# wkvong/multimodal-baby

Measured on AMD Instinct MI355X. Metric: image-text pairs/sec, CVCL ResNeXt+embed 224², bs256, 1/2/4/8 MI355X, higher is better.
Workload: dtype bf16; 1 GPU; C2 = BASELINE configs[1]: CVCL saycam_contrastive, frozen random-init ResNeXt-50 32x4d (BN train mode) + embedding mean-pool text encoder, E=512, L2-normalised, fixed tau 0.07, 224x224 frames + 3-word utterances; full step = fwd + InfoNCE + bwd(fc, embedding) + AdamW; per_gpu_batch=256, global_batch=256, negatives=local (single GPU), parallelism=dp1, trunk_streams=2

## Files before the change

multimodal-baby_amd/csrc/cvcl_common.h:

```cpp
#pragma once
#include <hip/hip_runtime.h>
#include <stdint.h>

#include "../../include/cvcl_hip.h"

typedef __bf16 bf16_t;
typedef __bf16 bf16x4 __attribute__((ext_vector_type(4)));
typedef __bf16 bf16x8 __attribute__((ext_vector_type(8)));
typedef float f32x4 __attribute__((ext_vector_type(4)));
typedef float f32x16 __attribute__((ext_vector_type(16)));
typedef unsigned int u32x4 __attribute__((ext_vector_type(4)));
typedef unsigned int u32x2 __attribute__((ext_vector_type(2)));

#define CVCL_WAVE 64

void cvcl_set_error(const char* fmt, ...);

int cvcl_gemm_cu_share();
bool cvcl_env_on(const char* name);

bool cvcl_prof_on();
void* cvcl_prof_begin(void* stream, int cls);
void cvcl_prof_end(void* handle, void* stream);
struct CvclProfScope {
    void* h; void* s;
    CvclProfScope(void* stream, int cls) : h(cvcl_prof_begin(stream, cls)), s(stream) {}
    ~CvclProfScope() { cvcl_prof_end(h, s); }
};

#ifdef __cplusplus
#include <atomic>
struct CvclLdsAttr {
    std::atomic<unsigned long long> devs{0};
    static int dev() { int d = 0; (void)hipGetDevice(&d); return d & 63; }
    bool ready() const { return (devs.load(std::memory_order_acquire) >> dev()) & 1ull; }
    void mark() { if (!ready()) devs.fetch_or(1ull << dev(), std::memory_order_release); }
};
static inline int cvcl_raise_lds_limit(CvclLdsAttr& attr, const void* kernel, int bytes, const char* entry) {
    if (attr.ready()) return CVCL_OK;
    if (hipFuncSetAttribute(kernel, hipFuncAttributeMaxDynamicSharedMemorySize, bytes) != hipSuccess) {
        cvcl_set_error("%s: cannot raise the dynamic LDS limit (%d bytes)", entry, bytes);
        return CVCL_ELAUNCH;
    }
    return CVCL_OK;
}
#endif

#define CVCL_CHECK_ARG(cond, ...)                \
    do {                                         \
        if (!(cond)) {                           \
            cvcl_set_error(__VA_ARGS__);         \
            return CVCL_EINVAL;                  \
        }                                        \
    } while (0)

#define CVCL_LAUNCH_CHECK()                                                    \
    do {                                                                       \
        hipError_t e_ = hipGetLastError();                                     \
        if (e_ != hipSuccess) {                                                \
            cvcl_set_error("%s:%d launch failed: %s", __FILE__, __LINE__,      \
                           hipGetErrorString(e_));                             \
            return CVCL_ELAUNCH;                                               \
        }                                                                      \
    } while (0)

__host__ __device__ static inline int cvcl_div_up(long a, long b) { return (int)((a + b - 1) / b); }

static inline int cvcl_grid(long items, int per_block, int cap) {
    const long g = (items + per_block - 1) / per_block;
    return (int)(g < 1 ? 1 : (g > cap ? cap : g));
}
static inline bool cvcl_aligned16(const void* p) { return ((uintptr_t)p & 15) == 0; }

static inline bool cvcl_dtype_plain(int d) { return d == CVCL_F32 || d == CVCL_BF16; }
static inline bool cvcl_dtype_trunk(int d) { return cvcl_dtype_plain(d) || d == CVCL_F32X3; }
static inline int cvcl_storage_dtype(int d) { return d == CVCL_F32X3 ? CVCL_F32 : d; }
#define CVCL_CHECK_DTYPE(d, fn) CVCL_CHECK_ARG(cvcl_dtype_plain(d), "%s: dtype %d is not accepted here (CVCL_F32 / CVCL_BF16)", fn, (int)(d))
#define CVCL_CHECK_DTYPE_TRUNK(d, fn) CVCL_CHECK_ARG(cvcl_dtype_trunk(d), "%s: unknown dtype %d", fn, (int)(d))

static inline bool cvcl_stats_rows_fit(const cvcl_gemm_args* a, int rows) {
    return !a->stats || a->stats_rows == CVCL_STATS_ACCUMULATE || a->stats_rows >= rows;
}
const char* cvcl_gemm8w_refusal(int epi, const cvcl_gemm_args* a, bool direct);
bool cvcl_gemm_pro_takes(const cvcl_gemm_args* a, bool stats);

constexpr int kSplitTerms = 6;
constexpr int kSplitParts = kSplitTerms == 3 ? 2 : 3;
int cvcl_gemm_split(const cvcl_gemm_args* a, void* stream);
int cvcl_gemm_split_stats_rows(int M, int N);
size_t cvcl_split_dense_bytes(long elems);
int cvcl_pack_split_dense(const float* w, void* out, long elems, void* stream);
size_t cvcl_split_conv_bytes(int stem, int cout);
int cvcl_pack_split_conv(int stem, const float* w, void* out, int cout, int cg, void* stream);
int cvcl_stem_split_stats_rows(int B, int H, int W);
int cvcl_gconv_split_stats_rows(int B, int H, int W, int C, int stride);
int cvcl_stem_split(const float* x, const void* w, float* y, float* stats, int stats_rows, const float* centre, int B, int H, int W,
                    void* stream);
int cvcl_gconv_split(const float* x, const float* a_scale, const float* a_shift, float act_floor, const void* w, float* y, float* stats,
                     int stats_rows, const float* centre, int B, int H, int W, int C, int cg, int stride, void* stream);

#ifdef __HIPCC__
template <typename T> struct ElemTraits;
template <> struct ElemTraits<float> {
    static constexpr int kPerChunk = 4;
    __device__ static inline float to_f(float v) { return v; }
    __device__ static inline float from_f(float v) { return v; }
};
template <> struct ElemTraits<bf16_t> {
    static constexpr int kPerChunk = 8;
    __device__ static inline float to_f(bf16_t v) { return (float)v; }
    __device__ static inline bf16_t from_f(float v) { return (bf16_t)v; }
};

template <typename T> struct Chunk;
template <> struct Chunk<float> {
    f32x4 v;
    __device__ inline void load(const float* p) { v = *reinterpret_cast<const f32x4*>(p); }
    __device__ inline void store(float* p) const { *reinterpret_cast<f32x4*>(p) = v; }
    __device__ inline void zero() { v = f32x4{0.f, 0.f, 0.f, 0.f}; }
    __device__ inline float get(int i) const { return v[i]; }
    __device__ inline void set(int i, float f) { v[i] = f; }
};
template <> struct Chunk<bf16_t> {
    bf16x8 v;
    __device__ inline void load(const bf16_t* p) { v = *reinterpret_cast<const bf16x8*>(p); }
    __device__ inline void store(bf16_t* p) const { *reinterpret_cast<bf16x8*>(p) = v; }
    __device__ inline void zero() {
        u32x4 z = {0u, 0u, 0u, 0u};
        v = __builtin_bit_cast(bf16x8, z);
    }
    __device__ inline float get(int i) const { return (float)v[i]; }
    __device__ inline void set(int i, float f) { v[i] = (bf16_t)f; }
};

typedef float f32x2 __attribute__((ext_vector_type(2)));
typedef __bf16 bf16x2 __attribute__((ext_vector_type(2)));
typedef short s16x2 __attribute__((ext_vector_type(2)));
__device__ __forceinline__ f32x2 widen2(unsigned u) {
    return f32x2{__builtin_bit_cast(float, u << 16), __builtin_bit_cast(float, u & 0xffff0000u)};
}
__device__ __forceinline__ float dot2c_bf16(float acc, unsigned a, unsigned b) {
    asm("v_dot2c_f32_bf16 %0, %1, %2" : "+v"(acc) : "v"(a), "v"(b));
    return acc;
}
template <int CTRL> __device__ __forceinline__ float dpp_quad_f32(float v) {
    return __builtin_bit_cast(float, __builtin_amdgcn_update_dpp(0, __builtin_bit_cast(int, v), CTRL, 0xf, 0xf, true));
}
__device__ __forceinline__ unsigned round2(f32x2 v) { return __builtin_bit_cast(unsigned, __builtin_convertvector(v, bf16x2)); }
__device__ __forceinline__ unsigned relu2(unsigned pair) {
    return __builtin_bit_cast(unsigned, __builtin_elementwise_max(__builtin_bit_cast(s16x2, pair), s16x2{0, 0}));
}

template <typename V> __device__ __forceinline__ void stream_store(V v, V* dst) { __builtin_nontemporal_store(v, dst); }

__device__ inline float wave_sum(float v) {
#pragma unroll
    for (int o = 32; o > 0; o >>= 1) v += __shfl_xor(v, o, 64);
    return v;
}
__device__ inline double wave_sum(double v) {
#pragma unroll
    for (int o = 32; o > 0; o >>= 1) v += __shfl_xor(v, o, 64);
    return v;
}
__device__ inline float wave_max(float v) {
#pragma unroll
    for (int o = 32; o > 0; o >>= 1) v = fmaxf(v, __shfl_xor(v, o, 64));
    return v;
}
__device__ __forceinline__ bool cvcl_better(float s, int i, float t, int j) { return s > t || (s == t && i < j); }
__device__ inline float block_sum(float v, float* scratch) {
    v = wave_sum(v);
    const int lane = threadIdx.x & 63, w = threadIdx.x >> 6, nw = (blockDim.x + 63) >> 6;
    __syncthreads();
    if (lane == 0) scratch[w] = v;
    __syncthreads();
    float r = 0.f;
    for (int i = 0; i < nw; ++i) r += scratch[i];
    return r;
}
__device__ inline float block_max(float v, float* scratch) {
    v = wave_max(v);
    const int lane = threadIdx.x & 63, w = threadIdx.x >> 6, nw = (blockDim.x + 63) >> 6;
    __syncthreads();
    if (lane == 0) scratch[w] = v;
    __syncthreads();
    float r = -INFINITY;
    for (int i = 0; i < nw; ++i) r = fmaxf(r, scratch[i]);
    return r;
}

constexpr int kBnAccRows = 8;
constexpr double kBnAccScale = 16777216.0;
__device__ __forceinline__ int cvcl_xcc_id() { return __builtin_amdgcn_s_getreg((3 << 11) | 20) & 7; }
constexpr long long kBnAccPoison = 1LL << 62;
constexpr float kBnAccMaxPartial = 268435456.f;
__device__ __forceinline__ void cvcl_bn_acc_add(float* stats_as_acc, int N, int n, float s, float q) {
    long long* row = reinterpret_cast<long long*>(stats_as_acc) + (long)cvcl_xcc_id() * 2 * N;
    if (fabsf(s) < kBnAccMaxPartial && fabsf(q) < kBnAccMaxPartial) {
        __hip_atomic_fetch_add(row + n, __double2ll_rn((double)s * kBnAccScale), __ATOMIC_RELAXED, __HIP_MEMORY_SCOPE_AGENT);
        __hip_atomic_fetch_add(row + N + n, __double2ll_rn((double)q * kBnAccScale), __ATOMIC_RELAXED, __HIP_MEMORY_SCOPE_AGENT);
    } else {
        __hip_atomic_fetch_max(row + N + n, kBnAccPoison, __ATOMIC_RELAXED, __HIP_MEMORY_SCOPE_AGENT);
    }
}
__device__ __forceinline__ void cvcl_bn_stats_out(float* stats, int acc_mode, long row, int N, int n, float s, float q) {
    if (acc_mode) cvcl_bn_acc_add(stats, N, n, s, q);
    else {
        stats[(row * 2 + 0) * N + n] = s;
        stats[(row * 2 + 1) * N + n] = q;
    }
}

__device__ inline float bn_ema(float r, float x, float m) { return fmaf(m, x, (1.f - m) * r); }

struct BnSrc {
    const long long* acc;
    int C;
    double count;
    const float* gamma; const float* beta; const float* centre;
    float* running_mean; float* running_var; int64_t* nbt;
    float momentum, eps;
    float* moments; int moments_ld;
    float* scale_out; float* shift_out;
};

template <int NCH>
__device__ __forceinline__ void bn_slice_affine(const BnSrc& b, int c0, bool publish, float* sc_out, float* sh_out) {
    const int c = threadIdx.x;
    if (c < NCH) {
        const int ch = c0 + c;
        long long v[2 * kBnAccRows];
#pragma unroll
        for (int r = 0; r < kBnAccRows; ++r) {
            v[2 * r] = b.acc[((long)r * 2 + 0) * b.C + ch];
            v[2 * r + 1] = b.acc[((long)r * 2 + 1) * b.C + ch];
        }
        long long S = 0, Q = 0;
        bool poisoned = false;
#pragma unroll
        for (int r = 0; r < kBnAccRows; ++r) { S += v[2 * r]; Q += v[2 * r + 1]; poisoned |= v[2 * r + 1] >= kBnAccPoison || v[2 * r + 1] < 0; }
        const double s = (double)S * (1.0 / kBnAccScale), q = (double)Q * (1.0 / kBnAccScale);
        const double mean = s / b.count;
        double var = q / b.count - mean * mean;
        if (var < 0.0) var = 0.0;
        if (poisoned) var = __builtin_nan("");
        const float sc = b.gamma[ch] / sqrtf((float)var + b.eps);
        const float sh = b.beta[ch] - (float)mean * sc;
        sc_out[c] = sc;
        sh_out[c] = sh;
        if (publish) {
            if (b.scale_out) { b.scale_out[ch] = sc; b.shift_out[ch] = sh; }
            const double unbiased = b.count > 1.0 ? var * b.count / (b.count - 1.0) : var;
            const float true_mean = b.centre ? (float)(mean + (double)b.centre[ch]) : (float)mean;
            if (b.moments) {
                b.moments[ch] = true_mean;
                b.moments[b.moments_ld + ch] = (float)unbiased;
            } else if (b.running_mean) {
                b.running_mean[ch] = bn_ema(b.running_mean[ch], true_mean, b.momentum);
                b.running_var[ch] = bn_ema(b.running_var[ch], (float)unbiased, b.momentum);
            }
        }
    }
    if (publish && !b.moments && b.nbt && c0 == 0 && threadIdx.x == 0) *b.nbt += 1;
    __syncthreads();
}

int cvcl_conv1x1_gram_src(const void* A, int lda, long M, int K, const float* a_scale, const float* a_shift, const BnSrc* src, int a_relu,
                          void* workspace, size_t workspace_bytes, const double** gram_out, void* stream);

template <int UN, typename ACC, typename F>
__device__ inline ACC ordered_sum(int n, F load) {
    ACC acc = (ACC)0;
    for (int i0 = 0; i0 < n; i0 += UN) {
        ACC v[UN];
#pragma unroll
        for (int u = 0; u < UN; ++u) v[u] = (ACC)load(min(i0 + u, n - 1));
#pragma unroll
        for (int u = 0; u < UN; ++u)
            if (i0 + u < n) acc += v[u];
    }
    return acc;
}

__device__ inline float gelu_erf_fast(float v) {
    const float x = fabsf(v) * 0.70710678118654752440f;
    const float t = __builtin_amdgcn_rcpf(fmaf(0.3275911f, x, 1.f));
    float poly = fmaf(1.061405429f, t, -1.453152027f);
    poly = fmaf(poly, t, 1.421413741f);
    poly = fmaf(poly, t, -0.284496736f);
    poly = fmaf(poly, t, 0.254829592f);
    poly *= t;
    const float e = __builtin_amdgcn_exp2f(-x * x * 1.4426950408889634f);
    const float erf_abs = fmaf(-poly, e, 1.f);
    return 0.5f * v * (1.f + copysignf(erf_abs, v));
}
__device__ inline float gelu_bf16out(float v) {
    const float u = fminf(v * v, 36.f);
    float p = fmaf(u, -0.0007030378797f * -1.4426950408889634f, 0.07401131995f * -1.4426950408889634f);
    p = fmaf(p, u, 1.595015736f * -1.4426950408889634f);
    const float e = __builtin_amdgcn_exp2f(v * p);
    return v * __builtin_amdgcn_rcpf(1.f + e);
}
__device__ inline f32x2 gelu_bf16out2(f32x2 v) {
    f32x2 u = v * v;
    u = f32x2{fminf(u[0], 36.f), fminf(u[1], 36.f)};
// ... 63 lines not shown
```

multimodal-baby_amd/csrc/gemm8w_kernel.h:

```cpp
#pragma once
#include <type_traits>

#include "cvcl_common.h"

namespace g8w {

constexpr int BN = 256;
constexpr int BK = 32;
constexpr int NSTAGE = 4;
constexpr int A_BYTES = 16384;
constexpr int STAGE_BYTES = 2 * A_BYTES;
constexpr int STG_BYTES = 2048;
constexpr int ACC_OFF = NSTAGE * STAGE_BYTES + 8 * STG_BYTES;
constexpr int LDS_BYTES = 160 * 1024;
constexpr int MAX_BIAS_N = (LDS_BYTES - ACC_OFF) / 4;

struct Dev {
    const bf16_t* A; const bf16_t* W; bf16_t* C; const bf16_t* R;
    const float* bias; float* stats;
    int stats_acc;
    const float* ln_stats; const float* ln_colsum; float* row_part;
    const float* centre;
    int M, N, K, lda, ldw, ldc, ldr, act;
    int tiles_m, grid_m, ncol;
    int gs, g_hw, g_wo, g_hi, g_wi;
    int a_rows;
};

__device__ __forceinline__ void glds16(const bf16_t* src, char* lds_wave_base) {
    __builtin_amdgcn_global_load_lds((const void __attribute__((address_space(1)))*)src,
                                     (void __attribute__((address_space(3)))*)lds_wave_base, 16, 0, 0);
}

__device__ __forceinline__ int swz(int g) { return (0x78 >> (2 * g)) & 3; }

template <int N> __device__ __forceinline__ void wait_vm() {
    static_assert(N >= 0 && N <= 63, "vmcnt is a 6-bit field");
    asm volatile("s_waitcnt vmcnt(%0)" ::"n"(N) : "memory");
}

__device__ __forceinline__ void wait_vm_value(int n, u32x4& v) {
#define CVCL_W(N) case N: asm volatile("s_waitcnt vmcnt(" #N ")" : "+v"(v) : : "memory"); break;
    switch (n) {
        CVCL_W(0) CVCL_W(1) CVCL_W(2) CVCL_W(3) CVCL_W(4) CVCL_W(5) CVCL_W(6) CVCL_W(7) CVCL_W(8) CVCL_W(9) CVCL_W(10) CVCL_W(11)
        CVCL_W(12) CVCL_W(13) CVCL_W(14) CVCL_W(15) CVCL_W(16) CVCL_W(17) CVCL_W(18) CVCL_W(19) CVCL_W(20) CVCL_W(21) CVCL_W(22)
        CVCL_W(23) CVCL_W(24) CVCL_W(25) CVCL_W(26) CVCL_W(27) CVCL_W(28) CVCL_W(29) CVCL_W(30) CVCL_W(31) CVCL_W(32) CVCL_W(33)
        CVCL_W(34) CVCL_W(35) CVCL_W(36) CVCL_W(37) CVCL_W(38) CVCL_W(39) CVCL_W(40)
        default: asm volatile("s_waitcnt vmcnt(0)" : "+v"(v) : : "memory"); break;
    }
#undef CVCL_W
}

template <int MI, int EPI, bool LNF, int ACT = CVCL_ACT_NONE>
__global__ __launch_bounds__(512, 2) void gemm8w_kernel(Dev p) {
    constexpr int BM = MI * 32;
    static_assert(!LNF || EPI >= 1, "LNF goes with the linear epilogues");
    static_assert(ACT == CVCL_ACT_NONE || EPI == 1, "activations go with the bias epilogue");
    constexpr int ESTORES = MI * 2 + (LNF && EPI == 2 ? MI * 2 : 0);
    extern __shared__ __attribute__((aligned(16))) char smem[];
    const int tid = threadIdx.x, lane = tid & 63;
    const int wave = __builtin_amdgcn_readfirstlane(tid >> 6);
    const int wm = wave >> 2, wn = wave & 3;

    constexpr bool LIN = EPI >= 1, RES = EPI == 2;
    constexpr bool FLAT = LIN;
    const int b = blockIdx.x;
    const int G = gridDim.x;
    int ti, tj, nt;
    int L0 = 0;
    const int cpx = G >> 3;
    auto decode = [&](int L, int& i_out, int& j_out) __attribute__((always_inline)) {
        const int per = p.grid_m * p.ncol;
        const int sr = L / per, rem = L - sr * per;
        const int ah = min(p.grid_m, p.tiles_m - sr * p.grid_m);
        const int col = rem / ah;
        i_out = sr * p.grid_m + (rem - col * ah);
        j_out = (sr & 1) ? p.ncol - 1 - col : col;
    };
    if constexpr (FLAT) {
        const int xcd = b & 7;
        const int total = p.tiles_m * p.ncol;
        const int S0 = (int)(((long)xcd * total) >> 3), S1 = (int)(((long)(xcd + 1) * total) >> 3);
        L0 = S0 + (b >> 3);
        nt = L0 < S1 ? (S1 - L0 + cpx - 1) / cpx : 0;
        ti = 0; tj = 0;
        if (nt > 0) decode(L0, ti, tj);
    } else {
        const int xcd = b & 7, s = b >> 3;
        tj = s % p.ncol;
        ti = (s / p.ncol) * 8 + xcd;
        nt = ti < p.tiles_m ? (p.tiles_m - ti + p.grid_m - 1) / p.grid_m : 0;
    }
    const int KS = p.K / BK;
    const int S = nt * KS;
    if (S == 0) {
        if (EPI == 0 && p.stats && !p.stats_acc && ti < p.grid_m && tid < BN) {
            p.stats[((long)ti * 2 + 0) * p.N + tj * BN + tid] = 0.f;
            p.stats[((long)ti * 2 + 1) * p.N + tj * BN + tid] = 0.f;
        }
        return;
    }
    const int step_i = p.grid_m;

    const bf16_t* __restrict__ A = p.A;
    const bf16_t* __restrict__ W = p.W;

    const int srow = lane >> 2;
    const int slog = (lane & 3) ^ swz((lane >> 4) & 3);
    unsigned w_off[2], a_raw[2];
#pragma unroll
    for (int j = 0; j < 2; ++j) {
        w_off[j] = (unsigned)(tj * BN + (wave * 2 + j) * 16 + srow) * (unsigned)p.ldw + slog * 8;
        int r = (wave * 2 + j) * 16 + srow;
        if (r >= BM) r = BM - 1;
        a_raw[j] = (unsigned)(ti * BM + r) * (unsigned)p.lda + slog * 8;
    }
    auto gathered = [&](int i_tile, int j) __attribute__((always_inline)) -> unsigned {
        int r = (wave * 2 + j) * 16 + srow;
        if (r >= BM) r = BM - 1;
        const unsigned m = (unsigned)min(i_tile * BM + r, p.M - 1);
        const unsigned bi = m / (unsigned)p.g_hw, rem = m - bi * (unsigned)p.g_hw;
        const unsigned oy = rem / (unsigned)p.g_wo, ox = rem - oy * (unsigned)p.g_wo;
        return ((bi * p.g_hi + oy * p.gs) * p.g_wi + ox * p.gs) * (unsigned)p.lda + slog * 8;
    };
    if (p.gs > 1) { a_raw[0] = gathered(ti, 0); a_raw[1] = gathered(ti, 1); }
    const unsigned a_unit = (unsigned)BM * (unsigned)p.lda;
    const unsigned a_lim = (unsigned)(p.a_rows - 1) * (unsigned)p.lda + 24;
    int l_t = 0, l_ks = 0, l_j = tj, l_i = ti;
    auto issue = [&](int buf) __attribute__((always_inline)) {
        char* base = smem + buf * STAGE_BYTES + wave * 2048;
        const int k0 = l_ks * BK;
#pragma unroll
        for (int j = 0; j < 2; ++j) glds16(A + min(a_raw[j], a_lim) + k0, base + j * 1024);
#pragma unroll
        for (int j = 0; j < 2; ++j) glds16(W + w_off[j] + k0, base + A_BYTES + j * 1024);
    };
    auto advance = [&]() __attribute__((always_inline)) {
        if constexpr (LNF && EPI == 1) {
            if (l_ks == 0 && wave < 4) {
                char* dst = smem + ACC_OFF + (l_t & 1) * 4096 + wave * 1024;
                const float* src = wave == 0 ? p.bias + l_j * BN + lane * 4 : wave == 1 ? p.ln_colsum + l_j * BN + lane * 4
                                 : p.ln_stats + (long)min(l_i * BM + (wave - 2) * 128 + lane * 2, (p.M - 1) & ~1) * 2;
                __builtin_amdgcn_global_load_lds((const void __attribute__((address_space(1)))*)src,
                                                 (void __attribute__((address_space(3)))*)dst, 16, 0, 0);
            }
        }
        if (++l_ks == KS) {
            l_ks = 0;
            if (l_t + 1 < nt) {
                ++l_t;
                if constexpr (FLAT) {
                    decode(L0 + l_t * cpx, l_i, l_j);
#pragma unroll
                    for (int j = 0; j < 2; ++j) {
                        const int rw = (wave * 2 + j) * 16 + srow;
                        a_raw[j] = (unsigned)(l_i * BM + min(rw, BM - 1)) * (unsigned)p.lda + slog * 8;
                        w_off[j] = (unsigned)(l_j * BN + rw) * (unsigned)p.ldw + slog * 8;
                    }
                } else {
                    l_i += step_i;
#pragma unroll
                    for (int j = 0; j < 2; ++j) {
                        if (p.gs > 1) a_raw[j] = gathered(l_i, j);
                        else a_raw[j] += (unsigned)step_i * a_unit;
                    }
                }
            }
        }
    };

    const int f_off = (lane & 15) * 64 + (((lane >> 4) ^ swz((lane >> 2) & 3)) << 4);
    const int a_base = wm * (BM / 2) * 64 + f_off;
    const int w_base = A_BYTES + wn * 64 * 64 + f_off;

    bf16x8 fa[2][MI], fw[2][4];
    f32x4 acc[4][MI];
    auto read_frags = [&](int buf, auto P) __attribute__((always_inline)) {
        constexpr int q = decltype(P)::value;
        const char* sb = smem + buf * STAGE_BYTES;
#pragma unroll
        for (int ni = 0; ni < 4; ++ni) fw[q][ni] = *reinterpret_cast<const bf16x8*>(sb + w_base + ni * 1024);
#pragma unroll
        for (int mi = 0; mi < MI; ++mi) fa[q][mi] = *reinterpret_cast<const bf16x8*>(sb + a_base + mi * 1024);
    };
    auto mma_half = [&](auto P, auto HALF) __attribute__((always_inline)) {
        constexpr int q = decltype(P)::value, h = decltype(HALF)::value;
#pragma unroll
        for (int ni = 2 * h; ni < 2 * h + 2; ++ni)
#pragma unroll
            for (int mi = 0; mi < MI; ++mi)
                acc[ni][mi] = __builtin_amdgcn_mfma_f32_16x16x32_bf16(fw[q][ni], fa[q][mi], acc[ni][mi], 0, 0, 0);
    };
#pragma unroll
    for (int ni = 0; ni < 4; ++ni)
#pragma unroll
        for (int mi = 0; mi < MI; ++mi) acc[ni][mi] = f32x4{0.f, 0.f, 0.f, 0.f};

    float* lds_acc = reinterpret_cast<float*>(smem + ACC_OFF);
    if constexpr (LIN && LNF && EPI == 1) {
    } else if constexpr (LIN) {
        for (int i = tid; i < p.N; i += 512) lds_acc[i] = p.bias ? p.bias[i] : 0.f;
    } else {
        lds_acc[tid] = 0.f;
        lds_acc[tid + 512] = 0.f;
// ... 226 lines not shown
```

multimodal-baby_amd/csrc/gemm_pro.hip:

```cpp
#include <cstdlib>

#include "cvcl_common.h"

namespace {

constexpr int PM = 64;
constexpr int PN = 256;

struct ProDev {
    const bf16_t* A; const bf16_t* W; bf16_t* C; const bf16_t* R;
    const float* a_scale; const float* a_shift; const float* c_scale; const float* c_shift; const float* r_scale; const float* r_shift;
    float* stats;
    int stats_acc;
    const float* centre;
    int M, N, lda, ldw, ldc, ldr;
    int tiles;
    const bf16_t* A2; const bf16_t* W2; const float* centre2;
    int lda2, ldw2;
};

enum { PRO_STATS = 0, PRO_STORE = 1, PRO_TAIL = 2, PRO_TAIL_DS = 3 };
constexpr int K2 = 64, KT2 = 2;
constexpr int X2BUF = PM * K2 * 2;

template <int KT> constexpr int pro_lds_bytes() { return 2 * PM * KT * 64 + 8 * 4096 + 6 * PN * 4 + 2 * 256 * 4 + 2 * X2BUF; }

template <int KT, int MODE, int D>
__global__ __launch_bounds__(512, 2) void gemm_pro_kernel(ProDev p) {
    constexpr bool TAIL = MODE == PRO_TAIL || MODE == PRO_TAIL_DS, DS = MODE == PRO_TAIL_DS;
    constexpr int K = KT * 32;
    constexpr int PITCH = K * 2;
    constexpr int CPR = K / 8;
    constexpr int NCH = PM * CPR / 512;
    constexpr int RPP = 512 / CPR;
    constexpr int ABUF = PM * PITCH;
    extern __shared__ __attribute__((aligned(16))) char smem[];
    const int tid = threadIdx.x, lane = tid & 63;
    const int wave = __builtin_amdgcn_readfirstlane(tid >> 6);
    const int wm = wave >> 2, wn = wave & 3;
    const int n0 = blockIdx.y * PN;

    bf16x8 fw[4][KT];
#pragma unroll
    for (int ni = 0; ni < 4; ++ni)
#pragma unroll
        for (int ks = 0; ks < KT; ++ks)
            fw[ni][ks] = *reinterpret_cast<const bf16x8*>(p.W + (long)(n0 + wn * 64 + ni * 16 + (lane & 15)) * p.ldw + ks * 32 + (lane >> 4) * 8);

    const int s_c = tid % CPR, s_r = tid / CPR;
    constexpr bool AFF_LDS = KT == 8;
    float* in_aff = reinterpret_cast<float*>(smem + 2 * ABUF + 8 * 4096 + 6 * PN * 4);
    char* x2buf = smem + 2 * ABUF + 8 * 4096 + 6 * PN * 4 + 2 * 256 * 4;
    const bool plain = p.a_scale == nullptr;
    const short fl = plain ? (short)-32768 : (short)0;
    const s16x2 floor2 = s16x2{fl, fl};
    f32x2 sc[4], sh[4];
#pragma unroll
    for (int e = 0; e < 4; ++e) { sc[e] = f32x2{1.f, 1.f}; sh[e] = f32x2{0.f, 0.f}; }
    if constexpr (AFF_LDS) {
        if (tid < K) { in_aff[tid] = plain ? 1.f : p.a_scale[tid]; in_aff[K + tid] = plain ? 0.f : p.a_shift[tid]; }
        __syncthreads();
    } else if (!plain) {
#pragma unroll
        for (int e = 0; e < 4; ++e) {
            sc[e] = f32x2{p.a_scale[s_c * 8 + 2 * e], p.a_scale[s_c * 8 + 2 * e + 1]};
            sh[e] = f32x2{p.a_shift[s_c * 8 + 2 * e], p.a_shift[s_c * 8 + 2 * e + 1]};
        }
    }
    u32x4 araw[D][NCH];
    auto load_a = [&](int tile, int slot) __attribute__((always_inline)) {
#pragma unroll
        for (int i = 0; i < NCH; ++i) {
            int m = tile * PM + s_r + RPP * i;
            if (m >= p.M) m = p.M - 1;
            araw[slot][i] = *reinterpret_cast<const u32x4*>(p.A + (long)m * p.lda + s_c * 8);
        }
    };
    auto stage_a = [&](int buf, int slot) __attribute__((always_inline)) {
        char* dst = smem + buf * ABUF;
        if constexpr (AFF_LDS) {
#pragma unroll
            for (int e = 0; e < 4; ++e) {
                sc[e] = *reinterpret_cast<const f32x2*>(in_aff + s_c * 8 + 2 * e);
                sh[e] = *reinterpret_cast<const f32x2*>(in_aff + K + s_c * 8 + 2 * e);
            }
        }
#pragma unroll
        for (int i = 0; i < NCH; ++i) {
            const int r = s_r + RPP * i;
            u32x4 v;
#pragma unroll
            for (int e = 0; e < 4; ++e) {
                const unsigned y = round2(__builtin_elementwise_fma(widen2(araw[slot][i][e]), sc[e], sh[e]));
                v[e] = __builtin_bit_cast(unsigned, __builtin_elementwise_max(__builtin_bit_cast(s16x2, y), floor2));
            }
            *reinterpret_cast<u32x4*>(dst + r * PITCH + ((s_c ^ (r & 15)) << 4)) = v;
        }
    };
    const int f_row = lane & 15, f_kc = lane >> 4;

    const int r_chunk = lane & 7, r_row0 = lane >> 3;
    float* aff = reinterpret_cast<float*>(smem + 2 * ABUF + 8 * 4096);
    if (tid < PN) aff[4 * PN + tid] = p.centre ? -p.centre[n0 + tid] : 0.f;
    if constexpr (DS) { if (tid < PN) aff[5 * PN + tid] = p.centre2 ? -p.centre2[n0 + tid] : 0.f; }
    const float* cen = aff + 4 * PN + wn * 64 + (lane >> 4) * 4;
    bf16x8 fw2[DS ? 4 : 1][DS ? KT2 : 1];
    u32x4 x2raw[DS ? D : 1];
    const int x_r = tid >> 3, x_c = tid & 7;
    if constexpr (DS) {
#pragma unroll
        for (int ni = 0; ni < 4; ++ni)
#pragma unroll
            for (int ks = 0; ks < KT2; ++ks)
                fw2[ni][ks] = *reinterpret_cast<const bf16x8*>(p.W2 + (long)(n0 + wn * 64 + ni * 16 + (lane & 15)) * p.ldw2 + ks * 32 + (lane >> 4) * 8);
    }
    auto load_x2 = [&](int tile, int slot) __attribute__((always_inline)) {
        int m = tile * PM + x_r;
        if (m >= p.M) m = p.M - 1;
        x2raw[slot] = *reinterpret_cast<const u32x4*>(p.A2 + (long)m * p.lda2 + x_c * 8);
    };
    auto stage_x2 = [&](int buf, int slot) __attribute__((always_inline)) {
        *reinterpret_cast<u32x4*>(x2buf + buf * X2BUF + x_r * 128 + ((x_c ^ (x_r & 7)) << 4)) = x2raw[slot];
    };
    if constexpr (TAIL) {
        if (tid < PN) {
            aff[tid] = p.c_scale[n0 + tid];
            aff[PN + tid] = p.c_shift[n0 + tid];
            aff[2 * PN + tid] = p.r_scale ? p.r_scale[n0 + tid] : 1.f;
            aff[3 * PN + tid] = p.r_scale ? p.r_shift[n0 + tid] : 0.f;
        }
    }
    bf16x8 rres[4];
    auto load_r = [&](int tile) __attribute__((always_inline)) {
#pragma unroll
        for (int j = 0; j < 4; ++j) {
            int m = tile * PM + wm * 32 + j * 8 + r_row0;
            if (m >= p.M) m = p.M - 1;
            rres[j] = *reinterpret_cast<const bf16x8*>(p.R + (long)m * p.ldr + n0 + wn * 64 + r_chunk * 8);
        }
    };
    f32x2 st_sum[8], st_sq[8];
#pragma unroll
    for (int e = 0; e < 8; ++e) { st_sum[e] = f32x2{0.f, 0.f}; st_sq[e] = f32x2{0.f, 0.f}; }

    char* stg = smem + 2 * ABUF + wave * 4096;
    const int e_row = lane & 15, e_wchunk = lane >> 5, e_wsub = ((lane >> 4) & 1) * 8;

    const int first = blockIdx.x;
    const int G = gridDim.x;
#pragma unroll
    for (int d = 0; d < D; ++d)
        if (first + d * G < p.tiles) {
            load_a(first + d * G, d);
            if constexpr (DS) load_x2(first + d * G, d);
        }
    if constexpr (MODE == PRO_TAIL) {
        if (first < p.tiles) load_r(first);
    }
    f32x4 acc[4][2];
    auto tile_stats = [&](int m0) __attribute__((always_inline)) {
#pragma unroll
        for (int mi = 0; mi < 2; ++mi) {
            const unsigned keep = m0 + mi * 16 + e_row < p.M ? 0xffffffffu : 0u;
#pragma unroll
            for (int ni = 0; ni < 4; ++ni)
#pragma unroll
                for (int h = 0; h < 2; ++h) {
                    const f32x2 f = widen2(round2(f32x2{acc[ni][mi][2 * h], acc[ni][mi][2 * h + 1]}) & keep);
                    st_sum[ni * 2 + h] += f;
                    st_sq[ni * 2 + h] = __builtin_elementwise_fma(f, f, st_sq[ni * 2 + h]);
                }
        }
    };
    int buf = 0;
    for (int tile = first; tile < p.tiles;) {
#pragma unroll
      for (int slot = 0; slot < D; ++slot) {
        if (tile >= p.tiles) break;
        stage_a(buf, slot);
        if constexpr (DS) stage_x2(buf, slot);
        __syncthreads();
        const int next = tile + G;
        if (tile + D * G < p.tiles) {
            load_a(tile + D * G, slot);
            if constexpr (DS) load_x2(tile + D * G, slot);
        }
        unsigned r2[DS ? 4 : 1][2][2];
        if constexpr (DS) {
            f32x4 acc2[4][2];
            const float* cen2 = aff + 5 * PN + wn * 64 + (lane >> 4) * 4;
#pragma unroll
            for (int ni = 0; ni < 4; ++ni) {
                const f32x4 c4 = *reinterpret_cast<const f32x4*>(cen2 + ni * 16);
#pragma unroll
                for (int mi = 0; mi < 2; ++mi) acc2[ni][mi] = c4;
            }
            const char* xb = x2buf + buf * X2BUF + (wm * 32 + f_row) * 128;
#pragma unroll
            for (int ks = 0; ks < KT2; ++ks) {
                bf16x8 fx[2];
#pragma unroll
                for (int mi = 0; mi < 2; ++mi)
                    fx[mi] = *reinterpret_cast<const bf16x8*>(xb + mi * 16 * 128 + (((ks * 4 + f_kc) ^ (f_row & 7)) << 4));
#pragma unroll
                for (int ni = 0; ni < 4; ++ni)
#pragma unroll
                    for (int mi = 0; mi < 2; ++mi)
                        acc2[ni][mi] = __builtin_amdgcn_mfma_f32_16x16x32_bf16(fw2[ni][ks], fx[mi], acc2[ni][mi], 0, 0, 0);
            }
#pragma unroll
            for (int ni = 0; ni < 4; ++ni)
#pragma unroll
                for (int mi = 0; mi < 2; ++mi) {
                    r2[ni][mi][0] = round2(f32x2{acc2[ni][mi][0], acc2[ni][mi][1]});
                    r2[ni][mi][1] = round2(f32x2{acc2[ni][mi][2], acc2[ni][mi][3]});
                }
        }
#pragma unroll
        for (int ni = 0; ni < 4; ++ni) {
            const f32x4 c4 = *reinterpret_cast<const f32x4*>(cen + ni * 16);
#pragma unroll
            for (int mi = 0; mi < 2; ++mi) acc[ni][mi] = c4;
        }
        const char* ab = smem + buf * ABUF + (wm * 32 + f_row) * PITCH;
#pragma unroll
        for (int ks = 0; ks < KT; ++ks) {
            bf16x8 fa[2];
#pragma unroll
            for (int mi = 0; mi < 2; ++mi)
                fa[mi] = *reinterpret_cast<const bf16x8*>(ab + mi * 16 * PITCH + (((ks * 4 + f_kc) ^ f_row) << 4));
#pragma unroll
            for (int ni = 0; ni < 4; ++ni)
#pragma unroll
                for (int mi = 0; mi < 2; ++mi)
                    acc[ni][mi] = __builtin_amdgcn_mfma_f32_16x16x32_bf16(fw[ni][ks], fa[mi], acc[ni][mi], 0, 0, 0);
        }
        const int m0 = tile * PM + wm * 32;
        if constexpr (MODE == PRO_STATS) {
            tile_stats(m0);
        } else if constexpr (DS) {
#pragma unroll
            for (int ni = 0; ni < 4; ++ni) {
                const float* t = aff + wn * 64 + ni * 16 + (lane >> 4) * 4;
                const f32x4 cs = *reinterpret_cast<const f32x4*>(t), cb = *reinterpret_cast<const f32x4*>(t + PN);
                const f32x4 rs = *reinterpret_cast<const f32x4*>(t + 2 * PN), rb = *reinterpret_cast<const f32x4*>(t + 3 * PN);
#pragma unroll
                for (int mi = 0; mi < 2; ++mi) {
                    bf16x4 q;
#pragma unroll
                    for (int e = 0; e < 4; ++e) {
                        const float y = fmaf((float)(bf16_t)acc[ni][mi][e], cs[e], cb[e]);
                        const float idv = fmaf(widen2(r2[ni][mi][e >> 1])[e & 1], rs[e], rb[e]);
                        q[e] = (bf16_t)fmaxf(y + idv, 0.f);
                    }
                    const int row = mi * 16 + e_row, chunk = ni * 2 + e_wchunk;
                    *reinterpret_cast<bf16x4*>(stg + row * 128 + ((chunk ^ ((row >> 1) & 7)) << 4) + e_wsub) = q;
                }
            }
#pragma unroll
            for (int j = 0; j < 4; ++j) {
                const int row = j * 8 + r_row0;
                const bf16x8 v = *reinterpret_cast<const bf16x8*>(stg + row * 128 + ((r_chunk ^ ((row >> 1) & 7)) << 4));
                const int m = m0 + row, n = n0 + wn * 64 + r_chunk * 8;
                if (m < p.M) stream_store(v, reinterpret_cast<bf16x8*>(p.C + (long)m * p.ldc + n));
            }
        } else {
#pragma unroll
            for (int mi = 0; mi < 2; ++mi)
#pragma unroll
                for (int ni = 0; ni < 4; ++ni) {
                    const bf16x4 q = {(bf16_t)acc[ni][mi][0], (bf16_t)acc[ni][mi][1], (bf16_t)acc[ni][mi][2], (bf16_t)acc[ni][mi][3]};
                    const int row = mi * 16 + e_row, chunk = ni * 2 + e_wchunk;
                    *reinterpret_cast<bf16x4*>(stg + row * 128 + ((chunk ^ ((row >> 1) & 7)) << 4) + e_wsub) = q;
                }
            float cs[8], cb[8], rs[8], rb[8];
            if constexpr (MODE == PRO_TAIL) {
                const float* t = aff + wn * 64 + r_chunk * 8;
#pragma unroll
                for (int e = 0; e < 8; ++e) { cs[e] = t[e]; cb[e] = t[PN + e]; rs[e] = t[2 * PN + e]; rb[e] = t[3 * PN + e]; }
            }
#pragma unroll
            for (int j = 0; j < 4; ++j) {
                const int row = j * 8 + r_row0;
                bf16x8 v = *reinterpret_cast<const bf16x8*>(stg + row * 128 + ((r_chunk ^ ((row >> 1) & 7)) << 4));
                const int m = m0 + row, n = n0 + wn * 64 + r_chunk * 8;
                if (m < p.M) {
                    if constexpr (MODE == PRO_TAIL) {
                        const bf16x8 r = rres[j];
#pragma unroll
                        for (int e = 0; e < 8; ++e) {
                            const float y = fmaf((float)v[e], cs[e], cb[e]);
                            const float idv = fmaf((float)r[e], rs[e], rb[e]);
                            v[e] = (bf16_t)fmaxf(y + idv, 0.f);
                        }
                    } else {
                        const u32x4 u = __builtin_bit_cast(u32x4, v);
#pragma unroll
                        for (int e = 0; e < 4; ++e) {
                            const f32x2 f = widen2(u[e]);
                            st_sum[e] += f;
                            st_sq[e] = __builtin_elementwise_fma(f, f, st_sq[e]);
                        }
                    }
                    stream_store(v, reinterpret_cast<bf16x8*>(p.C + (long)m * p.ldc + n));
                }
            }
            if constexpr (MODE == PRO_TAIL) {
                if (next < p.tiles) load_r(next);
            }
        }
        buf ^= 1;
        tile += G;
      }
    }

    if (!TAIL && p.stats) {
        __syncthreads();
        float* red = (float*)smem;
        if constexpr (MODE == PRO_STATS) {
#pragma unroll
            for (int e = 0; e < 8; ++e)
#pragma unroll
                for (int h = 0; h < 2; ++h)
#pragma unroll
                    for (int o = 1; o < 16; o <<= 1) {
                        st_sum[e][h] += __shfl_xor(st_sum[e][h], o, 64);
                        st_sq[e][h] += __shfl_xor(st_sq[e][h], o, 64);
                    }
            if ((lane & 15) == 0) {
#pragma unroll
                for (int ni = 0; ni < 4; ++ni)
#pragma unroll
                    for (int e = 0; e < 4; ++e) {
                        red[(wave * 2 + 0) * 64 + ni * 16 + (lane >> 4) * 4 + e] = st_sum[ni * 2 + (e >> 1)][e & 1];
                        red[(wave * 2 + 1) * 64 + ni * 16 + (lane >> 4) * 4 + e] = st_sq[ni * 2 + (e >> 1)][e & 1];
                    }
            }
        } else {
#pragma unroll
            for (int e = 0; e < 4; ++e)
#pragma unroll
                for (int h = 0; h < 2; ++h)
#pragma unroll
                    for (int o = 8; o <= 32; o <<= 1) {
                        st_sum[e][h] += __shfl_xor(st_sum[e][h], o, 64);
                        st_sq[e][h] += __shfl_xor(st_sq[e][h], o, 64);
                    }
            if (lane < 8) {
#pragma unroll
                for (int e = 0; e < 8; ++e) {
                    red[(wave * 2 + 0) * 64 + lane * 8 + e] = st_sum[e >> 1][e & 1];
                    red[(wave * 2 + 1) * 64 + lane * 8 + e] = st_sq[e >> 1][e & 1];
                }
            }
        }
        __syncthreads();
        if (tid < PN) {
            const int wn_ = tid >> 6, c = tid & 63, n = n0 + tid;
            cvcl_bn_stats_out(p.stats, p.stats_acc, blockIdx.x, p.N, n, red[(wn_ * 2 + 0) * 64 + c] + red[((wn_ + 4) * 2 + 0) * 64 + c],
                              red[(wn_ * 2 + 1) * 64 + c] + red[((wn_ + 4) * 2 + 1) * 64 + c]);
        }
    }
}

int pro_num_cus() {
    static int n = 0;
    if (!n) {
        int dev = 0;
        if (hipGetDevice(&dev) != hipSuccess || hipDeviceGetAttribute(&n, hipDeviceAttributeMultiprocessorCount, dev) != hipSuccess || n <= 0)
            n = 256;
    }
    return n;
}

template <int KT, int MODE, int D>
int pro_launch(const ProDev& d, dim3 grid, hipStream_t stream) {
    static CvclLdsAttr attr;
    constexpr int lds = pro_lds_bytes<KT>();
    if (const int rc = cvcl_raise_lds_limit(attr, (const void*)gemm_pro_kernel<KT, MODE, D>, lds, "cvcl_gemm_pro")) return rc;
    attr.mark();
    hipLaunchKernelGGL((gemm_pro_kernel<KT, MODE, D>), grid, dim3(512), lds, stream, d);
    CVCL_LAUNCH_CHECK();
    return CVCL_OK;
}

}

bool cvcl_gemm_pro_takes(const cvcl_gemm_args* a, bool stats) {
    const bool plain = !a->a_scale && !a->a_shift;
    if (!plain && (!a->a_scale || !a->a_shift || !a->a_relu)) return false;
    if (plain && (a->c_scale || a->A2 || a->W2)) return false;
    if ((a->K != 128 && a->K != 256) || a->N % PN != 0 || a->M < 1) return false;
    if (a->lda % 8 || a->ldw % 8 || (a->C && a->ldc % 8) || a->gather_stride > 1 || a->exp_scale || a->bias || a->C_pre || a->G) return false;
    if (!cvcl_aligned16(a->A) || !cvcl_aligned16(a->W) || !cvcl_aligned16(a->C) || !cvcl_aligned16(a->R)) return false;
    if (a->c_scale && a->A2)
        return a->c_shift && !a->R && a->C && !stats && a->act == CVCL_ACT_RELU && a->W2 && a->K2 == K2 && a->K == 128 && a->r_scale &&
               a->r_shift && a->lda2 % 8 == 0 && a->ldw2 % 8 == 0 && cvcl_aligned16(a->A2) && cvcl_aligned16(a->W2);
    if (a->A2 || a->W2) return false;
    if (a->c_scale) return a->c_shift && a->R && a->C && !stats && a->ldr % 8 == 0 && a->act == CVCL_ACT_RELU &&
                           (a->r_scale == nullptr) == (a->r_shift == nullptr);
    return !a->R && a->act == CVCL_ACT_NONE && (a->C || stats);
}
extern "C" int cvcl_gemm_pro_supported(const cvcl_gemm_args* a) { return a && cvcl_gemm_pro_takes(a, a->stats != nullptr); }

extern "C" int cvcl_gemm_pro_stats_rows(int M, int N) {
    const int tiles = cvcl_div_up(M, PM), ncol = N / PN;
    int g = pro_num_cus() / (ncol > 0 ? ncol : 1);
    if (g < 1) g = 1;
    return g > tiles ? tiles : g;
}

extern "C" int cvcl_gemm_pro(const cvcl_gemm_args* a, void* stream) {
    CVCL_CHECK_ARG(cvcl_gemm_pro_supported(a), "cvcl_gemm_pro: unsupported argument block");
    ProDev d;
    d.A = (const bf16_t*)a->A; d.W = (const bf16_t*)a->W; d.C = (bf16_t*)a->C; d.R = (const bf16_t*)a->R;
    d.a_scale = a->a_scale; d.a_shift = a->a_shift; d.c_scale = a->c_scale; d.c_shift = a->c_shift;
    d.r_scale = a->r_scale; d.r_shift = a->r_shift; d.stats = a->stats; d.centre = a->centre;
    d.stats_acc = a->stats && a->stats_rows == CVCL_STATS_ACCUMULATE;
    d.M = a->M; d.N = a->N; d.lda = a->lda; d.ldw = a->ldw; d.ldc = a->ldc; d.ldr = a->ldr;
    d.A2 = (const bf16_t*)a->A2; d.W2 = (const bf16_t*)a->W2; d.centre2 = a->centre2; d.lda2 = a->lda2; d.ldw2 = a->ldw2;
    d.tiles = cvcl_div_up(a->M, PM);
    const int gx = cvcl_gemm_pro_stats_rows(a->M, a->N);
    CVCL_CHECK_ARG(cvcl_stats_rows_fit(a, gx), "cvcl_gemm_pro: stats_rows %d < %d", a->stats_rows, gx);
    dim3 grid(gx, a->N / PN);
    const int mode = a->c_scale ? (a->A2 ? PRO_TAIL_DS : PRO_TAIL) : (a->C ? PRO_STORE : PRO_STATS);
    CvclProfScope prof(stream, CVCL_K_GEMM_PRO);
    hipStream_t st = (hipStream_t)stream;
    if (mode == PRO_TAIL_DS)
        return pro_launch<4, PRO_TAIL_DS, 2>(d, grid, st);
    if (a->K == 128) {
        if (mode == PRO_TAIL) return pro_launch<4, PRO_TAIL, 3>(d, grid, st);
        if (mode == PRO_STORE) return pro_launch<4, PRO_STORE, 3>(d, grid, st);
        return pro_launch<4, PRO_STATS, 3>(d, grid, st);
    }
    if (mode == PRO_TAIL) return pro_launch<8, PRO_TAIL, 2>(d, grid, st);
    if (mode == PRO_STORE) return pro_launch<8, PRO_STORE, 2>(d, grid, st);
    return pro_launch<8, PRO_STATS, 2>(d, grid, st);
}
```

Before: 51830 pairs/s.

## Pin prefetched tiles in reserved VGPRs with fine-grained vmcnt waits in tail GEMM

For the KT=8 PRO_TAIL D=2 GEMM specialisation, prefetched A and residual loads go into hand-reserved high VGPRs via inline asm. Each chunk then waits with a per-chunk vmcnt instead of letting the compiler hold them in allocated registers. The kernel is capped at 104 compiler VGPRs so more waves or registers fit, and full tiles take a branch-free epilogue. This risks register clobbering, since the asm relies on the compiler never touching the reserved registers, and it adds complex vmcnt bookkeeping that must match the exact load order.

Result: no change. 51770 pairs/s, median of 2 (-0.1%).

```diff
diff --git a/multimodal-baby_amd/csrc/cvcl_common.h b/multimodal-baby_amd/csrc/cvcl_common.h
--- a/multimodal-baby_amd/csrc/cvcl_common.h
+++ b/multimodal-baby_amd/csrc/cvcl_common.h
@@ -152,6 +152,59 @@
 }
 
 template <typename V> __device__ __forceinline__ void stream_store(V v, V* dst) { __builtin_nontemporal_store(v, dst); }
+
+template <int N> __device__ __forceinline__ void wait_vm() {
+    static_assert(N >= 0 && N <= 63, "vmcnt is a 6-bit field");
+    asm volatile("s_waitcnt vmcnt(%0)" ::"n"(N) : "memory");
+}
+
+__device__ __forceinline__ void wait_vm_value(int n, u32x4& v) {
+#define CVCL_W(N) case N: asm volatile("s_waitcnt vmcnt(" #N ")" : "+v"(v) : : "memory"); break;
+    switch (n) {
+        CVCL_W(0) CVCL_W(1) CVCL_W(2) CVCL_W(3) CVCL_W(4) CVCL_W(5) CVCL_W(6) CVCL_W(7) CVCL_W(8) CVCL_W(9) CVCL_W(10) CVCL_W(11)
+        CVCL_W(12) CVCL_W(13) CVCL_W(14) CVCL_W(15) CVCL_W(16) CVCL_W(17) CVCL_W(18) CVCL_W(19) CVCL_W(20) CVCL_W(21) CVCL_W(22)
+        CVCL_W(23) CVCL_W(24) CVCL_W(25) CVCL_W(26) CVCL_W(27) CVCL_W(28) CVCL_W(29) CVCL_W(30) CVCL_W(31) CVCL_W(32) CVCL_W(33)
+        CVCL_W(34) CVCL_W(35) CVCL_W(36) CVCL_W(37) CVCL_W(38) CVCL_W(39) CVCL_W(40)
+        default: asm volatile("s_waitcnt vmcnt(0)" : "+v"(v) : : "memory"); break;
+    }
+#undef CVCL_W
+}
+__device__ __forceinline__ void wait_vm_count(int n) {
+#define CVCL_W(N) case N: asm volatile("s_waitcnt vmcnt(" #N ")" ::: "memory"); break;
+    switch (n) {
+        CVCL_W(0) CVCL_W(1) CVCL_W(2) CVCL_W(3) CVCL_W(4) CVCL_W(5) CVCL_W(6) CVCL_W(7) CVCL_W(8) CVCL_W(9) CVCL_W(10) CVCL_W(11)
+        CVCL_W(12) CVCL_W(13) CVCL_W(14) CVCL_W(15) CVCL_W(16) CVCL_W(17) CVCL_W(18) CVCL_W(19) CVCL_W(20) CVCL_W(21) CVCL_W(22)
+        CVCL_W(23) CVCL_W(24) CVCL_W(25) CVCL_W(26) CVCL_W(27) CVCL_W(28) CVCL_W(29) CVCL_W(30) CVCL_W(31) CVCL_W(32) CVCL_W(33)
+        CVCL_W(34) CVCL_W(35) CVCL_W(36) CVCL_W(37) CVCL_W(38) CVCL_W(39) CVCL_W(40)
+        default: asm volatile("s_waitcnt vmcnt(0)" ::: "memory"); break;
+    }
+#undef CVCL_W
+}
+
+__device__ __forceinline__ void cvcl_fixed_claim() { asm volatile("" ::: "v255"); }
+template <int R> __device__ __forceinline__ void load16_fixed_reg(const void* base, unsigned byte_off) {
+    static_assert(R >= 0 && R + 3 <= 255, "register slot");
+    asm volatile("global_load_dwordx4 v[%0:%1], %2, %3" ::"n"(R), "n"(R + 3), "v"(byte_off), "s"(base) : "memory");
+}
+template <int R> __device__ __forceinline__ u32x4 take16_fixed_reg() {
+    unsigned long lo, hi;
+    asm volatile("v_mov_b64 %0, v[%2:%3]\n\tv_mov_b64 %1, v[%4:%5]" : "=v"(lo), "=v"(hi) : "n"(R), "n"(R + 1), "n"(R + 2), "n"(R + 3) : "memory");
+    return u32x4{(unsigned)lo, (unsigned)(lo >> 32), (unsigned)hi, (unsigned)(hi >> 32)};
+}
+#define CVCL_SLOTS(X) X(0) X(1) X(2) X(3) X(4) X(5) X(6) X(7) X(8) X(9) X(10) X(11)
+template <int R0> __device__ __forceinline__ void load16_fixed(int slot, const void* base, unsigned byte_off) {
+#define CVCL_S(N) case N: if constexpr (R0 + 4 * N + 3 <= 255) load16_fixed_reg<R0 + 4 * N>(base, byte_off); break;
+    switch (slot) { CVCL_SLOTS(CVCL_S) default: break; }
+#undef CVCL_S
+}
+template <int R0> __device__ __forceinline__ u32x4 take16_fixed(int slot) {
+    u32x4 v = {0u, 0u, 0u, 0u};
+#define CVCL_S(N) case N: if constexpr (R0 + 4 * N + 3 <= 255) v = take16_fixed_reg<R0 + 4 * N>(); break;
+    switch (slot) { CVCL_SLOTS(CVCL_S) default: break; }
+#undef CVCL_S
+    return v;
+}
+#undef CVCL_SLOTS
 
 __device__ inline float wave_sum(float v) {
 #pragma unroll
diff --git a/multimodal-baby_amd/csrc/gemm8w_kernel.h b/multimodal-baby_amd/csrc/gemm8w_kernel.h
--- a/multimodal-baby_amd/csrc/gemm8w_kernel.h
+++ b/multimodal-baby_amd/csrc/gemm8w_kernel.h
@@ -34,22 +34,6 @@
 
 __device__ __forceinline__ int swz(int g) { return (0x78 >> (2 * g)) & 3; }
 
-template <int N> __device__ __forceinline__ void wait_vm() {
-    static_assert(N >= 0 && N <= 63, "vmcnt is a 6-bit field");
-    asm volatile("s_waitcnt vmcnt(%0)" ::"n"(N) : "memory");
-}
-
-__device__ __forceinline__ void wait_vm_value(int n, u32x4& v) {
-#define CVCL_W(N) case N: asm volatile("s_waitcnt vmcnt(" #N ")" : "+v"(v) : : "memory"); break;
-    switch (n) {
-        CVCL_W(0) CVCL_W(1) CVCL_W(2) CVCL_W(3) CVCL_W(4) CVCL_W(5) CVCL_W(6) CVCL_W(7) CVCL_W(8) CVCL_W(9) CVCL_W(10) CVCL_W(11)
-        CVCL_W(12) CVCL_W(13) CVCL_W(14) CVCL_W(15) CVCL_W(16) CVCL_W(17) CVCL_W(18) CVCL_W(19) CVCL_W(20) CVCL_W(21) CVCL_W(22)
-        CVCL_W(23) CVCL_W(24) CVCL_W(25) CVCL_W(26) CVCL_W(27) CVCL_W(28) CVCL_W(29) CVCL_W(30) CVCL_W(31) CVCL_W(32) CVCL_W(33)
-        CVCL_W(34) CVCL_W(35) CVCL_W(36) CVCL_W(37) CVCL_W(38) CVCL_W(39) CVCL_W(40)
-        default: asm volatile("s_waitcnt vmcnt(0)" : "+v"(v) : : "memory"); break;
-    }
-#undef CVCL_W
-}
 
 template <int MI, int EPI, bool LNF, int ACT = CVCL_ACT_NONE>
 __global__ __launch_bounds__(512, 2) void gemm8w_kernel(Dev p) {
diff --git a/multimodal-baby_amd/csrc/gemm_pro.hip b/multimodal-baby_amd/csrc/gemm_pro.hip
--- a/multimodal-baby_amd/csrc/gemm_pro.hip
+++ b/multimodal-baby_amd/csrc/gemm_pro.hip
@@ -1,4 +1,5 @@
 #include <cstdlib>
+#include <type_traits>
 
 #include "cvcl_common.h"
 
@@ -25,9 +26,10 @@
 
 template <int KT> constexpr int pro_lds_bytes() { return 2 * PM * KT * 64 + 8 * 4096 + 6 * PN * 4 + 2 * 256 * 4 + 2 * X2BUF; }
 
-template <int KT, int MODE, int D>
-__global__ __launch_bounds__(512, 2) void gemm_pro_kernel(ProDev p) {
+template <int KT, int MODE, int D, int NV>
+__device__ __forceinline__ void gemm_pro_body(const ProDev& p) {
     constexpr bool TAIL = MODE == PRO_TAIL || MODE == PRO_TAIL_DS, DS = MODE == PRO_TAIL_DS;
+    constexpr bool CW = NV != 0;
     constexpr int K = KT * 32;
     constexpr int PITCH = K * 2;
     constexpr int CPR = K / 8;
@@ -67,16 +69,31 @@
             sh[e] = f32x2{p.a_shift[s_c * 8 + 2 * e], p.a_shift[s_c * 8 + 2 * e + 1]};
         }
     }
-    u32x4 araw[D][NCH];
+    constexpr int NA = NCH + (DS ? 1 : 0), NS = MODE == PRO_STATS ? 0 : 4, NR = MODE == PRO_TAIL ? 4 : 0;
+    constexpr int SLOT_X = D * NCH, SLOT_R = SLOT_X + (DS ? D : 0), NFIX = SLOT_R + NR, FIX0 = 256 - 4 * NFIX;
+    static_assert(!CW || 2 * NV == FIX0, "the compiler's registers end where the reserved ones begin");
+    if constexpr (CW) cvcl_fixed_claim();
+    u32x4 araw[CW ? 1 : D][CW ? 1 : NCH];
     auto load_a = [&](int tile, int slot) __attribute__((always_inline)) {
+        if constexpr (!CW) {
+#pragma unroll
+            for (int i = 0; i < NCH; ++i) {
+                int m = tile * PM + s_r + RPP * i;
+                if (m >= p.M) m = p.M - 1;
+                araw[slot][i] = *reinterpret_cast<const u32x4*>(p.A + (long)m * p.lda + s_c * 8);
+            }
+            return;
+        }
+        tile = min(tile, p.tiles - 1);
+        const int last = p.M - 1 - tile * PM;
+        const bf16_t* base = p.A + (long)tile * PM * p.lda;
 #pragma unroll
         for (int i = 0; i < NCH; ++i) {
-            int m = tile * PM + s_r + RPP * i;
-            if (m >= p.M) m = p.M - 1;
-            araw[slot][i] = *reinterpret_cast<const u32x4*>(p.A + (long)m * p.lda + s_c * 8);
-        }
-    };
-    auto stage_a = [&](int buf, int slot) __attribute__((always_inline)) {
+            const int li = last - RPP * i;
+            load16_fixed<FIX0>(slot * NCH + i, base + (long)(li >= 0 ? RPP * i : last) * p.lda, (unsigned)(min(s_r, max(li, 0)) * p.lda + s_c * 8) * 2u);
+        }
+    };
+    auto stage_a = [&](int buf, int slot, int younger) __attribute__((always_inline)) {
         char* dst = smem + buf * ABUF;
         if constexpr (AFF_LDS) {
 #pragma unroll
@@ -88,10 +105,17 @@
 #pragma unroll
         for (int i = 0; i < NCH; ++i) {
             const int r = s_r + RPP * i;
+            u32x4 raw;
+            if constexpr (CW) {
+                wait_vm_count(younger + NA - 1 - i);
+                raw = take16_fixed<FIX0>(slot * NCH + i);
+            } else {
+                raw = araw[slot][i];
+            }
             u32x4 v;
 #pragma unroll
             for (int e = 0; e < 4; ++e) {
-                const unsigned y = round2(__builtin_elementwise_fma(widen2(araw[slot][i][e]), sc[e], sh[e]));
+                const unsigned y = round2(__builtin_elementwise_fma(widen2(raw[e]), sc[e], sh[e]));
                 v[e] = __builtin_bit_cast(unsigned, __builtin_elementwise_max(__builtin_bit_cast(s16x2, y), floor2));
             }
             *reinterpret_cast<u32x4*>(dst + r * PITCH + ((s_c ^ (r & 15)) << 4)) = v;
@@ -105,7 +129,6 @@
     if constexpr (DS) { if (tid < PN) aff[5 * PN + tid] = p.centre2 ? -p.centre2[n0 + tid] : 0.f; }
     const float* cen = aff + 4 * PN + wn * 64 + (lane >> 4) * 4;
     bf16x8 fw2[DS ? 4 : 1][DS ? KT2 : 1];
-    u32x4 x2raw[DS ? D : 1];
     const int x_r = tid >> 3, x_c = tid & 7;
     if constexpr (DS) {
 #pragma unroll
@@ -114,13 +137,20 @@
             for (int ks = 0; ks < KT2; ++ks)
                 fw2[ni][ks] = *reinterpret_cast<const bf16x8*>(p.W2 + (long)(n0 + wn * 64 + ni * 16 + (lane & 15)) * p.ldw2 + ks * 32 + (lane >> 4) * 8);
     }
+    u32x4 x2raw[DS && !CW ? D : 1];
     auto load_x2 = [&](int tile, int slot) __attribute__((always_inline)) {
-        int m = tile * PM + x_r;
-        if (m >= p.M) m = p.M - 1;
-        x2raw[slot] = *reinterpret_cast<const u32x4*>(p.A2 + (long)m * p.lda2 + x_c * 8);
-    };
-    auto stage_x2 = [&](int buf, int slot) __attribute__((always_inline)) {
-        *reinterpret_cast<u32x4*>(x2buf + buf * X2BUF + x_r * 128 + ((x_c ^ (x_r & 7)) << 4)) = x2raw[slot];
+        if constexpr (!CW) {
+            int m = tile * PM + x_r;
+            if (m >= p.M) m = p.M - 1;
+            x2raw[slot] = *reinterpret_cast<const u32x4*>(p.A2 + (long)m * p.lda2 + x_c * 8);
+            return;
+        }
+        tile = min(tile, p.tiles - 1);
+        load16_fixed<FIX0>(SLOT_X + slot, p.A2 + (long)tile * PM * p.lda2, (unsigned)(min(x_r, p.M - 1 - tile * PM) * p.lda2 + x_c * 8) * 2u);
+    };
+    auto stage_x2 = [&](int buf, int slot, int younger) __attribute__((always_inline)) {
+        if constexpr (CW) wait_vm_count(younger);
+        *reinterpret_cast<u32x4*>(x2buf + buf * X2BUF + x_r * 128 + ((x_c ^ (x_r & 7)) << 4)) = CW ? take16_fixed<FIX0>(SLOT_X + slot) : x2raw[slot];
     };
     if constexpr (TAIL) {
         if (tid < PN) {
@@ -130,13 +160,24 @@
             aff[3 * PN + tid] = p.r_scale ? p.r_shift[n0 + tid] : 0.f;
         }
     }
-    bf16x8 rres[4];
+    u32x4 rres[CW ? 1 : 4];
     auto load_r = [&](int tile) __attribute__((always_inline)) {
+        if constexpr (!CW) {
+#pragma unroll
+            for (int j = 0; j < 4; ++j) {
+                int m = tile * PM + wm * 32 + j * 8 + r_row0;
+                if (m >= p.M) m = p.M - 1;
+                rres[j] = *reinterpret_cast<const u32x4*>(p.R + (long)m * p.ldr + n0 + wn * 64 + r_chunk * 8);
+            }
+            return;
+        }
+        tile = min(tile, p.tiles - 1);
+        const int last = p.M - 1 - tile * PM;
+        const bf16_t* base = p.R + (long)tile * PM * p.ldr + n0 + wn * 64;
 #pragma unroll
         for (int j = 0; j < 4; ++j) {
-            int m = tile * PM + wm * 32 + j * 8 + r_row0;
-            if (m >= p.M) m = p.M - 1;
-            rres[j] = *reinterpret_cast<const bf16x8*>(p.R + (long)m * p.ldr + n0 + wn * 64 + r_chunk * 8);
+            const int lj = last - wm * 32 - j * 8;
+            load16_fixed<FIX0>(SLOT_R + j, base + (long)(lj >= 0 ? wm * 32 + j * 8 : last) * p.ldr, (unsigned)(min(r_row0, max(lj, 0)) * p.ldr + r_chunk * 8) * 2u);
         }
     };
     f32x2 st_sum[8], st_sq[8];
@@ -148,14 +189,15 @@
 
     const int first = blockIdx.x;
     const int G = gridDim.x;
+    if constexpr (CW) __builtin_amdgcn_s_waitcnt(0x0F70);
 #pragma unroll
     for (int d = 0; d < D; ++d)
-        if (first + d * G < p.tiles) {
+        if (CW || first + d * G < p.tiles) {
             load_a(first + d * G, d);
             if constexpr (DS) load_x2(first + d * G, d);
         }
     if constexpr (MODE == PRO_TAIL) {
-        if (first < p.tiles) load_r(first);
+        if (CW || first < p.tiles) load_r(first);
     }
     f32x4 acc[4][2];
     auto tile_stats = [&](int m0) __attribute__((always_inline)) {
@@ -172,16 +214,25 @@
                 }
         }
     };
+    auto stage = [&](int buf, int slot, bool first_round) __attribute__((always_inline)) {
+        const int steady = D * (NS + NR) + (D - 1) * NA, start = (D - 1) * NA + NR + slot * (NS + NR);
+        if (first_round) {
+            stage_a(buf, slot, start);
+            if constexpr (DS) stage_x2(buf, slot, start);
+        } else {
+            stage_a(buf, slot, steady);
+            if constexpr (DS) stage_x2(buf, slot, steady);
+        }
+    };
     int buf = 0;
     for (int tile = first; tile < p.tiles;) {
 #pragma unroll
       for (int slot = 0; slot < D; ++slot) {
         if (tile >= p.tiles) break;
-        stage_a(buf, slot);
-        if constexpr (DS) stage_x2(buf, slot);
+        stage(buf, slot, tile < first + D * G);
         __syncthreads();
         const int next = tile + G;
-        if (tile + D * G < p.tiles) {
+        if (CW || tile + D * G < p.tiles) {
             load_a(tile + D * G, slot);
             if constexpr (DS) load_x2(tile + D * G, slot);
         }
@@ -236,6 +287,8 @@
                     acc[ni][mi] = __builtin_amdgcn_mfma_f32_16x16x32_bf16(fw[ni][ks], fa[mi], acc[ni][mi], 0, 0, 0);
         }
         const int m0 = tile * PM + wm * 32;
+        auto epilogue = [&](auto FULL) __attribute__((always_inline)) {
+        constexpr bool full = decltype(FULL)::value;
         if constexpr (MODE == PRO_STATS) {
             tile_stats(m0);
         } else if constexpr (DS) {
@@ -262,7 +315,7 @@
                 const int row = j * 8 + r_row0;
                 const bf16x8 v = *reinterpret_cast<const bf16x8*>(stg + row * 128 + ((r_chunk ^ ((row >> 1) & 7)) << 4));
                 const int m = m0 + row, n = n0 + wn * 64 + r_chunk * 8;
-                if (m < p.M) stream_store(v, reinterpret_cast<bf16x8*>(p.C + (long)m * p.ldc + n));
+                if (full || m < p.M) stream_store(v, reinterpret_cast<bf16x8*>(p.C + (long)m * p.ldc + n));
             }
         } else {
 #pragma unroll
@@ -274,19 +327,25 @@
                     *reinterpret_cast<bf16x4*>(stg + row * 128 + ((chunk ^ ((row >> 1) & 7)) << 4) + e_wsub) = q;
                 }
             float cs[8], cb[8], rs[8], rb[8];
-            if constexpr (MODE == PRO_TAIL) {
+            auto load_aff = [&]() __attribute__((always_inline)) {
                 const float* t = aff + wn * 64 + r_chunk * 8;
 #pragma unroll
                 for (int e = 0; e < 8; ++e) { cs[e] = t[e]; cb[e] = t[PN + e]; rs[e] = t[2 * PN + e]; rb[e] = t[3 * PN + e]; }
-            }
+            };
+            constexpr bool AFF_PER_GROUP = CW && AFF_LDS;
+            if constexpr (MODE == PRO_TAIL && !AFF_PER_GROUP) load_aff();
 #pragma unroll
             for (int j = 0; j < 4; ++j) {
                 const int row = j * 8 + r_row0;
                 bf16x8 v = *reinterpret_cast<const bf16x8*>(stg + row * 128 + ((r_chunk ^ ((row >> 1) & 7)) << 4));
                 const int m = m0 + row, n = n0 + wn * 64 + r_chunk * 8;
-                if (m < p.M) {
+                if constexpr (MODE == PRO_TAIL && CW) {
+                    wait_vm_count(full ? (3 - j) + NA + j : 0);
+                }
+                if (full || m < p.M) {
                     if constexpr (MODE == PRO_TAIL) {
-                        const bf16x8 r = rres[j];
+                        if constexpr (AFF_PER_GROUP) load_aff();
+                        const bf16x8 r = __builtin_bit_cast(bf16x8, CW ? take16_fixed<FIX0>(SLOT_R + j) : rres[j]);
 #pragma unroll
                         for (int e = 0; e < 8; ++e) {
                             const float y = fmaf((float)v[e], cs[e], cb[e]);
@@ -305,15 +364,19 @@
                     stream_store(v, reinterpret_cast<bf16x8*>(p.C + (long)m * p.ldc + n));
                 }
             }
-            if constexpr (MODE == PRO_TAIL) {
-                if (next < p.tiles) load_r(next);
-            }
+        }
+        };
+        if (CW && (tile + 1) * PM <= p.M) epilogue(std::true_type{});
+        else epilogue(std::false_type{});
+        if constexpr (MODE == PRO_TAIL) {
+            if (CW || next < p.tiles) load_r(next);
         }
         buf ^= 1;
         tile += G;
       }
     }
 
+    if constexpr (CW) wait_vm<0>();
     if (!TAIL && p.stats) {
         __syncthreads();
         float* red = (float*)smem;
@@ -361,6 +424,13 @@
                               red[(wn_ * 2 + 1) * 64 + c] + red[((wn_ + 4) * 2 + 1) * 64 + c]);
         }
     }
+}
+
+template <int KT, int MODE, int D>
+__global__ __launch_bounds__(512, 2) void gemm_pro_kernel(ProDev p) { gemm_pro_body<KT, MODE, D, 0>(p); }
+template <>
+__global__ __launch_bounds__(512, 2) __attribute__((amdgpu_num_vgpr(104))) void gemm_pro_kernel<8, PRO_TAIL, 2>(ProDev p) {
+    gemm_pro_body<8, PRO_TAIL, 2, 104>(p);
 }
 
 int pro_num_cus() {
@@ -391,6 +461,7 @@
     if (!plain && (!a->a_scale || !a->a_shift || !a->a_relu)) return false;
     if (plain && (a->c_scale || a->A2 || a->W2)) return false;
     if ((a->K != 128 && a->K != 256) || a->N % PN != 0 || a->M < 1) return false;
+    if (a->lda >= 1 << 24 || a->ldr >= 1 << 24 || a->lda2 >= 1 << 24) return false;
     if (a->lda % 8 || a->ldw % 8 || (a->C && a->ldc % 8) || a->gather_stride > 1 || a->exp_scale || a->bias || a->C_pre || a->G) return false;
     if (!cvcl_aligned16(a->A) || !cvcl_aligned16(a->W) || !cvcl_aligned16(a->C) || !cvcl_aligned16(a->R)) return false;
     if (a->c_scale && a->A2)
```
